# xiyichen/smplify-x-partial

Measured on AMD Instinct MI355X. Metric: fitted frames/sec, higher is better.
Workload: dtype f32; 1 GPU; configs[1]: 256 synthetic frames/GPU, body-only K=25, camera + 5-stage L-BFGS (fit_smplx_smplifyx.yaml, use_vposer=False); frames_per_gpu=256, lbs_mode=dense, gemm_columns_per_gpu=256, parallelism=frames sharded, dp1, closure_evals_per_frame_max=4429, non_finite=0

## Files before the change

smplify-x-partial_amd/csrc/closure_body.h:

```cpp
#pragma once
#include "closure_math.h"
#include "closure_lds.h"
#pragma clang fp contract(on)

#define MARK(i) do { if (D.dbg && blockIdx.x == 0 && threadIdx.x == 0 && D.dbg[62] <= D.dbg[61]) { D.dbg[i] = clock64(); \
        if ((i) == 0) D.dbg[17] = wall_clock64(); if ((i) == 16) D.dbg[18] = wall_clock64(); } } while (0)

#define FOR_CT(w, N) _Pragma("unroll") for (int w##_i = 0; w##_i < ((N) + CT - 1) / CT; ++w##_i)             \
                         if (const int w = t + w##_i * CT; w < (N))

struct NoUpstream {};
struct ExtUpstream {
    const float* djoints;
    int has_dverts;
    float* gc;
};

template <class LDS, class SW, class EXT = NoUpstream>
__device__ __forceinline__ void closure_body(LDS& S, const DevModel& M, const BatchDev& D,
                                             const VarList* __restrict__ vls, const SW* __restrict__ sws,
                                             const ClosureArgs& args, const int b, typename LDS::real_t* gflat,
                                             typename LDS::real_t* fout, const EXT& ext = EXT{}) {
    using Real = typename LDS::real_t;
    constexpr bool F64 = std::is_same<Real, double>::value;
    constexpr bool kExt = !std::is_same<EXT, NoUpstream>::value;
    static_assert(!kExt || !F64, "the external-upstream sweep is fp32");
    constexpr int CT = LDS::kThreads;
    const int t = threadIdx.x;
    const int lane = t & 63, wv = t >> 6;
    const ParLayout& L = D.L;
    const BatchCfgDev& C = D.cfg;

    const bool self_uvp = !F64 && args.use_dense_verts == 2 && M.n_uniq > 0 && M.n_uniq <= LDS::kMaxItems;
    const int stage = __builtin_amdgcn_readfirstlane((args.stage_override != -2) ? args.stage_override : D.stage[b]);
    if constexpr (!kExt) { if (stage >= C.n_stages && !args.forward_only) return; }
    const bool cam_stage = (stage < 0);
    const SW sw = (kExt || cam_stage || args.forward_only) ? SW{} : sws[stage];

    const int cls = (kExt || cam_stage || args.forward_only) ? 2 : ((sw.face_jw != 0.f) ? 2 : ((sw.hand_jw != 0.f) ? 1 : 0));
    const int KL = __builtin_amdgcn_readfirstlane(cls == 2 ? M.K : C.kl[cls]);
    const int NIL = __builtin_amdgcn_readfirstlane(cls == 2 ? M.n_items : C.nil[cls]);

    MARK(0);
    constexpr bool HAS_VP = !std::is_same<decltype(S.V), EmptyLDS>::value;
    constexpr int RIF = (LDS::kMaxItems <= SFX_SMALL_ITEMS) ? SFX_RIF_SMALL : SFX_RIF_BIG;
    constexpr int FWD_PREFIX = (int)(offsetof(LDS, vp) / sizeof(float));
    static_assert(F64 || (FWD_PREFIX % 4 == 0 && FWD_PREFIX + 96 + 2 * VP_H + 128 + 64 <= SFX_FWD_N), "forward-state blob layout");
    static_assert(offsetof(LDS, Ad) % sizeof(fwd_t) == 0 && offsetof(LDS, cd) % sizeof(fwd_t) == 0, "forward-precision members");
    const bool reuse = !F64 && args.reuse_fwd != 0;
    float* fwd = D.fwd ? D.fwd + (size_t)b * SFX_FWD_N : nullptr;
    const Real* xsrc;
// ... 12 lines not shown
    lds_fill_async<CT>(S.vt, M.item_vt, ns * 3);
    lds_fill_async<CT>(S.wj, M.item_wj, ns * SFX_NW); lds_fill_async<CT>(S.ww, M.item_ww, ns * SFX_NW);
    if (M.n_sj <= LDS::kMaxItems * SFX_NW) {
        lds_fill_async<CT>(S.sjs, M.sj_start, SFX_J + 1);
        lds_fill_async<CT>(S.sji, M.sj_item, M.n_sj); lds_fill_async<CT>(S.sjw, M.sj_w, M.n_sj);
    }
    }
    if (reuse) {
        static_assert(F64 || offsetof(LDS, lut_row) == offsetof(LDS, lh45) + 2 * SFX_NHAND * sizeof(float), "hand poses + LUT row are one run");
        lds_fill_async16<CT>(&S, fwd, FWD_PREFIX / 4);
        const float* ex = fwd + FWD_PREFIX;
        lds_fill_async<CT>(S.lh45, ex, 2 * SFX_NHAND + 1);
        if constexpr (HAS_VP) if (C.use_vposer) {
            const float* vx = ex + 96;
            static_assert(offsetof(VposerLDS, h2) == VP_H * sizeof(float) && offsetof(VposerLDS, o) == 2 * VP_H * sizeof(float), "h1 | h2 | o are one run");
            lds_fill_async16<CT>(S.V.h1, vx, (2 * VP_H + 128) / 4);
            lds_fill_async16<CT>(S.V.body, vx + 2 * VP_H + 128, 64 / 4);
        }
    }
    for (int i = t; i < SFX_KD_PAD; i += CT) { if (!reuse) S.feat[i] = 0.f; S.dfeat[i] = 0.f; }
    for (int i = t; i < SFX_NPAR_MAX; i += CT) S.gc[i] = 0.f;
    for (int i = t; i < 168; i += CT) S.dpose[i] = 0.f;
    if constexpr (!F64) {
        if (self_uvp) self_blend_offsets(M.uniq_dirs, M.n_uniq, D.featR + (size_t)args.self_col * SFX_KD_PAD, S.dvert, wv, CT / 64, lane);
    }
    lds_dma_wait();
    __syncthreads();
    const Real* bodypose = S.x + L.emb;
    if constexpr (HAS_VP) {
        if (C.use_vposer && !reuse) {
            vposer_forward<CT>(S.V, M, S.x + L.emb, S.T);
            if (t < 63) D.bodypose[(size_t)b * 63 + t] = S.V.body[t];
        }
        if (C.use_vposer) bodypose = S.V.body;
    }
  if (!reuse) {

    MARK(1);
    if (t < SFX_POSE) {
        Real v;
        if (t < 3) v = S.x[L.go + t];
        else if (t < 66) v = bodypose[t - 3];
        else if (t < 69) v = S.x[L.jaw + t - 66];
        else if (t < 72) v = S.x[L.leye + t - 69];
        else if (t < 75) v = S.x[L.reye + t - 72];
        else {
            const bool left = t < 120;
// ... 91 lines not shown
            for (int q = 0; q < 5; ++q) {
                const Real* Rk = &S.R[chain[q] * 9];
                float o[9];
                for (int i = 0; i < 3; ++i)
                    for (int j = 0; j < 3; ++j)
                        o[i * 3 + j] = Rk[i * 3] * rel[j] + Rk[i * 3 + 1] * rel[3 + j] + Rk[i * 3 + 2] * rel[6 + j];
                for (int e = 0; e < 9; ++e) rel[e] = o[e];
            }
            const float sy = sqrtf(rel[0] * rel[0] + rel[3] * rel[3]);
            const float ang = atan2f(-rel[6], sy);
            float deg = (-ang) * 180.0f / 3.14159265358979323846f;
            deg = fminf(deg, 39.f);
            const int y = (int)rintf(deg);
            row = (y < -39) ? 78 : ((y < 0) ? (39 - y) : y);
        }
        S.lut_row = row;
    }
    __syncthreads();

  }
    MARK(4);
    if (!F64 && args.export_dense) {
        const int slot = D.slot[b];
        if (t < SFX_KD_PAD / 4) reinterpret_cast<float4*>(D.featR_w + (size_t)slot * SFX_KD_PAD)[t] = reinterpret_cast<const float4*>(S.feat)[t];
        MARK(17);
        for (int i = t; i < SFX_J * 12; i += CT) {
            const int j = i / 12, e = i % 12;
            D.AT_w[((size_t)e * SFX_JPAD + j) * D.Bpad + slot] = S.A[i];
        }
        MARK(18);
        if (args.forward_only == 2) {
            if (fwd) {
                const float* sp = reinterpret_cast<const float*>(&S);
                for (int i = t; i < FWD_PREFIX / 4; i += CT)
                    reinterpret_cast<float4*>(fwd)[i] = reinterpret_cast<const float4*>(sp)[i];
                float* ex = fwd + FWD_PREFIX;
                if (t < SFX_NHAND) { ex[t] = S.lh45[t]; ex[SFX_NHAND + t] = S.rh45[t]; }
                if (t == 64) ex[2 * SFX_NHAND] = __int_as_float(S.lut_row);
                if constexpr (HAS_VP) if (C.use_vposer) {
                    float* vx = ex + 96;
                    for (int i = t; i < VP_H; i += CT) { vx[i] = S.V.h1[i]; vx[VP_H + i] = S.V.h2[i]; }
                    if (t < 128) vx[2 * VP_H + t] = S.V.o[t];
                    if (t < 64) vx[2 * VP_H + 128 + t] = S.V.body[t];
                }
            }
            MARK(19);
            return;
        }
    }

    MARK(5);
// ... 604 lines not shown
```

smplify-x-partial_amd/csrc/fused.hip:

```cpp
#include "closure_body.h"
#include "lbfgs_body.h"

#ifndef SFX_SETS_SMALL8
#define SFX_SETS_SMALL8 3
#endif
#ifndef SFX_TICK_OCC
#define SFX_TICK_OCC 2
#endif

template <class LDS>
__global__ __launch_bounds__(LDS::kThreads, LDS::kBlocksPerCU)
void k_fit_rows(DevModel M, BatchDev D, const VarList* __restrict__ vls, const StageW* __restrict__ sws,
                int first_stage, int last_stage, int max_ticks) {
    __shared__ LDS S;
    __shared__ float gflat[SFX_NVAR_MAX];
    __shared__ float fval;
    __shared__ float s_al[SFX_HIST_MAX + 2 * LB_BS];
    __shared__ OptScal st;
    const int b = blockIdx.x;
    ClosureArgs a{};
    a.stage_override = -2;
    for (int it = 0; it < max_ticks; ++it) {
        if (D.stage[b] > last_stage) break;
        closure_body(S, M, D, vls, sws, a, b, gflat, &fval);
// ... 67 lines not shown
            if (D.pen_want && threadIdx.x == 0) D.pen_want[D.slot[b]] = 0;
            copy_operand_column(D, D.slot[b], CTK);
            return;
        }
    }
    const int stage_now = (PF && has_eval) ? s_stage : D.stage[b];
    if (D.pen_want && threadIdx.x == 0) {
        const int st_ = stage_now;
        D.pen_want[D.slot[b]] = (st_ >= 0 && st_ < D.cfg.n_stages) ? (sws[st_].coll > 0.f ? 1 : 0) : 0;
    }
    ClosureArgs e{};
    e.stage_override = -2; e.export_dense = 1; e.forward_only = 2; e.keep_tables = has_eval;
    if (PF && has_eval) { e.stage_override = stage_now; e.x_lds = s_pf + NVEC * SFX_NVAR_MAX + SFX_NPAR_MAX; }
    closure_body(S, M, D, vls, sws, e, b, nullptr, nullptr);
    if (D.dbg && b == 0 && threadIdx.x == 0 && D.dbg[62] <= D.dbg[61]) D.dbg[26] = clock64();
    if (D.dbg && threadIdx.x == 0) {
        const long long dt = wall_clock64() - wc0;
        atomicMax((unsigned long long*)&D.dbg[58], (unsigned long long)dt);
        atomicAdd((unsigned long long*)&D.dbg[59], (unsigned long long)dt);
        atomicAdd((unsigned long long*)&D.dbg[60], 1ull);
    }
}

__global__ __launch_bounds__(256)
void k_uvp_self(DevModel M, BatchDev D, float* __restrict__ out) {
    const int col = blockIdx.x;
    self_blend_offsets(M.uniq_dirs, M.n_uniq, D.featR + (size_t)col * SFX_KD_PAD, out + (size_t)col * M.n_uniq * 3,
                       threadIdx.x >> 6, 4, threadIdx.x & 63);
}
void launch_uvp_self(const DevModel& M, const BatchDev& D, float* out, hipStream_t s) {
    if (D.cfg.B <= 0 || M.n_uniq <= 0) return;
    hipLaunchKernelGGL(k_uvp_self, dim3(D.cfg.B), dim3(256), 0, s, M, D, out);
}

void launch_fit_rows(const DevModel& M, const BatchDev& D, const VarList* vl_dev, const StageW* sw_dev,
                     int first_stage, int last_stage, int max_ticks, hipStream_t s) {
    if (sfx_small_closure(M, D))
        hipLaunchKernelGGL(k_fit_rows<FrameLDSSmall>, dim3(D.cfg.B), dim3(FrameLDSSmall::kThreads), 0, s, M, D, vl_dev, sw_dev, first_stage, last_stage, max_ticks);
    else
        hipLaunchKernelGGL(k_fit_rows<FrameLDS>, dim3(D.cfg.B), dim3(FrameLDS::kThreads), 0, s, M, D, vl_dev, sw_dev, first_stage, last_stage, max_ticks);
}
void launch_tick_dense(const DevModel& M, const BatchDev& D, const VarList* vl_dev, const StageW* sw_dev,
                       int first_stage, int last_stage, int has_eval, hipStream_t s) {
    const int grid = D.act ? D.nrun : D.cfg.B;
    if (grid <= 0) return;
    static const int n_cu = [] { hipDeviceProp_t p; int dev = 0; (void)hipGetDevice(&dev); return hipGetDeviceProperties(&p, dev) == hipSuccess ? p.multiProcessorCount : 256; }();
    if (sfx_small_closure(M, D)) {
#ifdef SFX_LAB
        static const bool t256 = [] { const char* e = getenv("SFX_TICK_THREADS"); return e && atoi(e) == 256; }();
#else
        constexpr bool t256 = false;
#endif
        if (grid <= n_cu && !t256)
            hipLaunchKernelGGL((k_tick_dense<FrameLDSSmall8, 1>), dim3(grid), dim3(FrameLDSSmall8::kThreads), 0, s, M, D, vl_dev, sw_dev, first_stage, last_stage, has_eval);
        else if (grid <= n_cu)
            hipLaunchKernelGGL((k_tick_dense<FrameLDSSmall, 1>), dim3(grid), dim3(FrameLDSSmall::kThreads), 0, s, M, D, vl_dev, sw_dev, first_stage, last_stage, has_eval);
        else
            hipLaunchKernelGGL((k_tick_dense<FrameLDSSmall, SFX_TICK_OCC>), dim3(grid), dim3(FrameLDSSmall::kThreads), 0, s, M, D, vl_dev, sw_dev, first_stage, last_stage, has_eval);
    } else
        hipLaunchKernelGGL((k_tick_dense<FrameLDS, 1>), dim3(grid), dim3(FrameLDS::kThreads), 0, s, M, D, vl_dev, sw_dev, first_stage, last_stage, has_eval);
}
```

smplify-x-partial_amd/csrc/host/batch.hip:

```cpp
#include "host.h"

#include <cmath>
#include <memory>

static void build_layout(ParLayout& L, int NB, int NE, int NPCA, int use_vposer, int latent) {
    L.NB = NB; L.NE = NE; L.NPCA = NPCA;
    L.cam_t = 0; L.go = 3; L.betas = 6; L.lh = L.betas + NB; L.rh = L.lh + NPCA; L.expr = L.rh + NPCA;
    L.jaw = L.expr + NE; L.leye = L.jaw + 3; L.reye = L.leye + 3; L.bodyp = L.reye + 3;
    L.has_bodyp = use_vposer ? 0 : 1;
    L.emb = L.bodyp + (L.has_bodyp ? 63 : 0);
    L.NEMB = use_vposer ? latent : 63;
    L.npar = L.emb + L.NEMB;
}

static void add_group(VarList& v, int off, int len, int has) {
    const int g = v.ngroups++;
    v.g_off[g] = (short)v.n; v.g_len[g] = (short)len; v.g_has[g] = (short)has;
    for (int i = 0; i < len; ++i, ++v.n) if (v.n < SFX_NVAR_MAX) v.idx[v.n] = (short)(off + i);
}

template <class W, class S>
static std::vector<W> stage_weights(const S* st, int n, bool coll) {
    using T = decltype(W::bpw);
    std::vector<W> out(std::max(1, n));
// ... 78 lines not shown
    D.X = b->mem.zeros<float>((size_t)B * SFX_NPAR_MAX);
    D.Xt = b->mem.zeros<float>((size_t)B * SFX_NPAR_MAX);
    if (b->f64) {
        D.X64 = b->mem.zeros<double>((size_t)B * SFX_NPAR_MAX);
        D.Xt64 = b->mem.zeros<double>((size_t)B * SFX_NPAR_MAX);
        D.f64 = b->mem.zeros<double>(B);
        D.g64 = b->mem.zeros<double>((size_t)B * SFX_NVAR_MAX);
        D.cam64 = b->mem.zeros<double>((size_t)B * 8);
    }
    D.gt = b->mem.zeros<float>((size_t)B * K * 2);
    D.conf = b->mem.zeros<float>((size_t)B * K);
    D.jw = b->mem.zeros<float>((size_t)B * K);
    D.cmask = b->mem.zeros<float>((size_t)B * K);
    D.cam = b->mem.zeros<float>((size_t)B * 8);
    D.camR = b->mem.zeros<float>((size_t)B * 9);
    D.regpose = b->mem.zeros<float>((size_t)B * 63);
    D.fd = b->mem.zeros<float>((size_t)B * FD_N);
    D.f = b->mem.zeros<float>(B);
    D.g = b->mem.zeros<float>((size_t)B * SFX_NVAR_MAX);
    D.bodypose = b->mem.zeros<float>((size_t)B * 63);
    D.featR = b->mem.zeros<float>((size_t)SFX_KD_PAD * D.Bpad);
    D.AT = b->mem.zeros<float>((size_t)12 * SFX_JPAD * D.Bpad);
    D.featR_w = D.featR; D.AT_w = D.AT;
    if (c->lbs_mode == 1 && !D.cfg.pen) {
        for (int i = 0; i < 2; ++i) {
            b->featR_o[i] = b->mem.zeros<float>((size_t)SFX_KD_PAD * D.Bpad);
            b->AT_o[i] = b->mem.zeros<float>((size_t)12 * SFX_JPAD * D.Bpad);
        }
    }
    D.verts = b->mem.zeros<float>((size_t)B * m->M.V * 3);
    D.fwd = b->mem.zeros<float>((size_t)B * SFX_FWD_N);
    D.uvp = b->mem.zeros<float>((size_t)B * std::max(1, m->M.n_uniq) * 3);
    if (D.cfg.pen) {
        const int F = (int)(m->faces_host.size() / 3);
        const bool parts = !m->segm_host.empty();
        const int pen_cols = (c->slots > 0 && c->slots < B && c->lbs_mode == 1) ? std::min(B, ((c->slots + 31) / 32) * 32) : B;
        const int pen_cap = std::max(1, c->max_collisions);
        b->pen = m->pen_idle.take(pen_cols, pen_cap, m->parts_gen, &b->pen_cols);
        if (b->pen) sfx_pen_reuse(b->pen);
        else {
            int rc = sfx_pen_create(m->M.V, F, m->faces_host.data(), parts ? m->segm_host.data() : nullptr,
                                    parts ? m->parents_host.data() : nullptr, m->ign_host.empty() ? nullptr : m->ign_host.data(),
                                    (int)(m->ign_host.size() / 2), pen_cap, pen_cols, &b->pen);
            if (rc) return rc;
            b->pen_cols = pen_cols;
        }
        b->pen_cap = pen_cap; b->pen_gen = m->parts_gen;
        b->pen_sigma = c->df_cone_height; b->pen_outside = c->penalize_outside ? 1 : 0;
        (void)sfx_pen_set_point2plane(b->pen, c->point2plane);
        D.pen_loss = b->mem.zeros<float>(B);
// ... 263 lines not shown
```

smplify-x-partial_amd/csrc/host/fit_loop.hip:

```cpp
#include "host.h"
#include "../column_pool.h"

#include <chrono>
#include <cstdio>
#include <cstdlib>
#include <cstring>

static long sfx_fit_tick_bound(const BatchCfgDev& c, int first_stage, int last_stage) {
    const long per_step = (long)c.max_eval + std::max(25, (int)c.lbfgs_max_iter) + 1;
    return (long)(last_stage - first_stage + 1) * c.maxiters * std::max(80L, per_step + 7) * 2  * 2  + 64;
}

struct DenseSwitches {
    bool dbg_nact = false, dbg_host = false;
    int rpb = 0, ahead = 0;
    bool ov_on = true, self_on = true, self_in_serial = false;
    int ov_serial = SFX_OV_SERIAL, self_serial = SFX_OV_SELF_SERIAL, self_max = SFX_OV_SELF_MAX;
};
static const DenseSwitches& dense_switches() {
#ifdef SFX_LAB
    static const DenseSwitches w = [] {
        const auto num = [](const char* name, int unset) { const char* e = getenv(name); return e && *e ? atoi(e) : unset; };
        DenseSwitches v;
        v.dbg_nact = getenv("SFX_DEBUG_NACT") != nullptr; v.dbg_host = getenv("SFX_DEBUG_HOST") != nullptr;
        v.rpb = num("SFX_POLL_ROUNDS", 0); v.ahead = num("SFX_POLL_AHEAD", 0);
        v.ov_on = num("SFX_DENSE_OVERLAP", 1) != 0; v.self_on = num("SFX_DENSE_SELF", 1) != 0; v.self_in_serial = num("SFX_DENSE_SELF_SERIAL", 0) != 0;
        v.ov_serial = num("SFX_OVERLAP_SERIAL", SFX_OV_SERIAL); v.self_max = num("SFX_DENSE_SELF_MAX", SFX_OV_SELF_MAX);
        v.self_serial = num("SFX_OVERLAP_SERIAL", SFX_OV_SELF_SERIAL);
        return v;
    }();
#else
    static constexpr DenseSwitches w{};
#endif
    return w;
}

namespace {
struct DenseLoop {
    sfx_batch* const b; const hipStream_t s; const int first_stage, last_stage;
    BatchDev& D = b->D; const DevModel& M = b->m->M; const int B = D.cfg.B;
    bool overlap = false, self_form = false;
    hipEvent_t last_G = nullptr, prev_G = nullptr;
    hipEvent_t last_T = nullptr;
    long ov_i = 0, tick = 0;
    ColumnPool pool;
    int upl = 0, rpb = 8;
    double host_enq_s = 0.0, host_wait_s = 0.0; long host_batches = 0;
    static inline long nact_hist[9] = {};
    void tick_kernel(const char* name, const BatchDev& Dx, int has_eval) {
        ProfScope p(name, s, Dx.nrun);
        launch_tick_dense(M, Dx, b->vl_dev, b->sw_dev, first_stage, last_stage, has_eval, s);
    }
    int join_s2() {
        if (last_G) SFX_CHECK(hipStreamWaitEvent(s, last_G, 0));
        last_G = prev_G = nullptr;
        return 0;
    }
    int upload(const std::vector<int>* fresh) {
        const std::vector<int>& run = pool.run;
        int* h = b->map_host + (size_t)upl * 3 * B; upl = (upl + 1) % SFX_POLL_BUFS;
        memcpy(h, pool.col.data(), (size_t)B * sizeof(int));
        memcpy(h + B, run.data(), run.size() * sizeof(int));
        SFX_CHECK(hipMemcpyAsync(D.slot, h, (size_t)B * sizeof(int), hipMemcpyHostToDevice, s));
        if (!run.empty()) SFX_CHECK(hipMemcpyAsync(b->act_dev, h + B, run.size() * sizeof(int), hipMemcpyHostToDevice, s));
        if (fresh && !fresh->empty()) {
            memcpy(h + 2 * B, fresh->data(), fresh->size() * sizeof(int));
            SFX_CHECK(hipMemcpyAsync(b->act_new_dev, h + 2 * B, fresh->size() * sizeof(int), hipMemcpyHostToDevice, s));
        }
        D.act = b->act_dev; D.nrun = (int)run.size();
        return 0;
    }
    int tick_beside(hipEvent_t e_G, int has_eval) {
        if (prev_G) SFX_CHECK(hipStreamWaitEvent(s, prev_G, 0));
        prev_G = last_G; last_G = e_G;
        BatchDev Dt = D; Dt.featR_w = b->featR_o[0]; Dt.AT_w = b->AT_o[0];
        tick_kernel("tick", Dt, has_eval);
        float* const f = D.featR; D.featR = b->featR_o[0]; b->featR_o[0] = b->featR_o[1]; b->featR_o[1] = f;
        float* const a = D.AT; D.AT = b->AT_o[0]; b->AT_o[0] = b->AT_o[1]; b->AT_o[1] = a;
        D.featR_w = D.featR; D.AT_w = D.AT;
        return 0;
    }
    int round_self() {
        const int k = (int)(ov_i++ % SFX_OV_EVENTS);
        if (!last_G || !last_T) { SFX_CHECK(hipEventRecord(b->ov_ev[0][k], s)); last_T = b->ov_ev[0][k]; }
        SFX_CHECK(hipStreamWaitEvent(b->s2, last_T, 0));
        { ProfScope p("lbs_dense", b->s2, D.nact); launch_lbs_dense(M, D, b->s2); }
        SFX_CHECK(hipEventRecord(b->ov_ev[1][k], b->s2));
        if (int rc = tick_beside(b->ov_ev[1][k], 2)) return rc;
        last_T = b->ov_ev[0][(k + 1) % SFX_OV_EVENTS];
        SFX_CHECK(hipEventRecord(last_T, s));
        return 0;
    }
    int round_key_rest() {
        if (last_T) { if (int rc = join_s2()) return rc; last_T = nullptr; }
        const int k = (int)(ov_i++ % SFX_OV_EVENTS);
        if (b->m->n_key) { ProfScope p("lbs_dense_key", s, D.nact); launch_lbs_dense_list(M, D, b->m->tile_key, b->m->n_key, s); }
        SFX_CHECK(hipEventRecord(b->ov_ev[0][k], s));
        SFX_CHECK(hipStreamWaitEvent(b->s2, b->ov_ev[0][k], 0));
        { ProfScope p("lbs_dense", b->s2, D.nact); launch_lbs_dense_list(M, D, b->m->tile_rest, b->m->n_rest, b->s2); }
        SFX_CHECK(hipEventRecord(b->ov_ev[1][k], b->s2));
        return tick_beside(b->ov_ev[1][k], 1);
    }
    int round_serial() {
        if (int rc = join_s2()) return rc;
        last_T = nullptr;
        { ProfScope p("lbs_dense", s, D.nact); launch_lbs_dense(M, D, s); }
        if (int rc = eval_penetration(b, -2, s, true)) return rc;
        tick_kernel("tick", D, (dense_switches().self_in_serial && !b->pen && M.n_uniq <= SFX_OV_SELF_UNIQ) ? 2 : 1);
        return 0;
    }
    int rounds(int buf) {
        const DenseSwitches& sw = dense_switches();
        if (sw.dbg_nact) nact_hist[std::min(8, (D.nact - 1) / 32)] += rpb;
        const auto h0 = std::chrono::steady_clock::now();
        for (int q = 0; q < rpb; ++q, ++tick) {
            const int rc = self_form && D.nact > sw.self_serial && D.nact <= sw.self_max ? round_self()
                         : overlap && D.nact > sw.ov_serial && D.nact <= SFX_OV_MAX      ? round_key_rest() : round_serial();
            if (rc) return rc;
        }
        SFX_CHECK(hipMemcpyAsync(b->stage_host + (size_t)buf * B, D.stage, (size_t)B * sizeof(int), hipMemcpyDeviceToHost, s));
        SFX_CHECK(hipEventRecord(b->poll_ev[buf], s));
        host_enq_s += std::chrono::duration<double>(std::chrono::steady_clock::now() - h0).count(); ++host_batches;
        return 0;
    }
    int poll(int cur, bool& done) {
        const auto w0 = std::chrono::steady_clock::now();
        SFX_CHECK(hipEventSynchronize(b->poll_ev[cur]));
        host_wait_s += std::chrono::duration<double>(std::chrono::steady_clock::now() - w0).count();
        std::vector<int> fresh;
        const bool changed = pool.retire(b->stage_host + (size_t)cur * B, last_stage, fresh);
        done = pool.run.empty();
        if (done || !changed) return 0;
        if (!fresh.empty()) {
            if (int rc = join_s2()) return rc;
            if (int rc = upload(&fresh)) return rc;
            BatchDev Dn = D; Dn.act = b->act_new_dev; Dn.nrun = (int)fresh.size();
            tick_kernel("tick_admit", Dn, 0);
        } else if (ColumnPool::slice_emptied(D.nact, (int)pool.run.size())) {
            D.nact = pool.compact();
            if (int rc = join_s2()) return rc;
            if (int rc = upload(nullptr)) return rc;
            tick_kernel("tick", D, 0);
        } else if (int rc = upload(nullptr)) return rc;
        return 0;
    }
    int run(long max_ticks, bool& done) {
        const DenseSwitches& sw = dense_switches();
        overlap = sw.ov_on && !b->pen && b->featR_o[0] && b->featR_o[1] && b->AT_o[0] && b->AT_o[1];
        if (overlap && !b->s2) {
            int lo = 0, hi = 0;
            SFX_CHECK(hipDeviceGetStreamPriorityRange(&lo, &hi));
            SFX_CHECK(hipStreamCreateWithPriority(&b->s2, hipStreamNonBlocking, lo));
            for (auto& ring : b->ov_ev) for (hipEvent_t& e : ring) SFX_CHECK(hipEventCreateWithFlags(&e, hipEventDisableTiming));
        }
        self_form = overlap && sw.self_on && M.n_uniq <= SFX_OV_SELF_UNIQ;
        {
            struct OvDrain { sfx_batch* b; hipStream_t s;
                             ~OvDrain() { if (b->s2) (void)hipStreamSynchronize(b->s2); (void)hipStreamSynchronize(s); b->D.featR_w = b->D.featR; b->D.AT_w = b->D.AT; } } ov_drain{b, s};
            const int ncol = b->slots > 0 ? std::min(b->slots, B) : B;
            pool.reset(B, ncol);
            D.nact = ncol;
            if (int rc = upload(nullptr)) return rc;
            tick_kernel("tick", D, 0);
            const double wall0 = std::chrono::duration<double>(std::chrono::steady_clock::now().time_since_epoch()).count();
            rpb = std::max(1, std::min(64, sw.rpb > 0 ? sw.rpb : 8));
            const int ahead = std::max(1, std::min(SFX_POLL_BUFS - 1, sw.ahead > 0 ? sw.ahead : (b->pen ? 1 : 3)));
            long q_head = 0, q_next = 0;
            for (; q_next < ahead; ++q_next) if (int rc = rounds((int)(q_next % SFX_POLL_BUFS))) return rc;
            while (!done && tick < max_ticks + (long)rpb * (ahead + 1)) {
                if (int rc = rounds((int)(q_next++ % SFX_POLL_BUFS))) return rc;
                if (int rc = poll((int)(q_head++ % SFX_POLL_BUFS), done)) return rc;
            }
            if (b->s2) SFX_CHECK(hipStreamSynchronize(b->s2));
            SFX_CHECK(hipStreamSynchronize(s));
            D.act = nullptr; D.nrun = 0;
            const double wall = std::chrono::duration<double>(std::chrono::steady_clock::now().time_since_epoch()).count() - wall0;
            loop_host_add(host_enq_s, host_wait_s, wall, (double)host_batches * rpb);
            if (sw.dbg_host)
                fprintf(stderr, "[sfx] host enqueue: %ld batches of rounds, %.1f us of host time per round, %.1f %% of the loop's %.1f ms wall time\n",
                        host_batches, 1e6 * host_enq_s / std::max(1L, host_batches * rpb), 100.0 * host_enq_s / std::max(wall, 1e-9), 1e3 * wall);
            if (sw.dbg_nact) {
                fprintf(stderr, "[sfx] rounds by active columns (<=32, <=64, ..., <=256, more), cumulative:");
                for (int i = 0; i < 9; ++i) fprintf(stderr, " %ld", nact_hist[i]);
                fprintf(stderr, "\n");
            }
        }
        SFX_CHECK(hipGetLastError());
        std::vector<int> id(B);
        for (int i = 0; i < B; ++i) id[i] = i;
// ... 73 lines not shown
```

smplify-x-partial_amd/csrc/host/host.h:

```cpp
#pragma once
#include "../../../include/sfx.h"
#include "../sfx_internal.h"
#include "../collide_host.h"
#include "idle_slot.h"

#include <map>
#include <vector>

struct sfx_model {
    DevModel M{};
    DevAlloc mem;
    std::vector<int> faces_host, segm_host, parents_host, ign_host;
    int NB = 0, NE = 0, NPCA = 0;
    std::vector<int> meta_host;
    const int *tile_key = nullptr, *tile_rest = nullptr;
    int n_key = 0, n_rest = 0;
    sfx_batch* fwd = nullptr;
    int fwd_B = 0;
    IdleSlot<sfx_pen, sfx_pen_destroy> pen_idle;
    int parts_gen = 0;
    ~sfx_model() { sfx_batch_destroy(fwd); pen_idle.drop(); }
};

#define SFX_POLL_BUFS 8
#define SFX_OV_EVENTS 4
#ifndef SFX_OV_MAX
#define SFX_OV_MAX 256
#endif
#ifndef SFX_OV_SERIAL
#define SFX_OV_SERIAL 160
#endif
#ifndef SFX_OV_SELF_SERIAL
#define SFX_OV_SELF_SERIAL 64
#endif
#ifndef SFX_OV_SELF_MAX
#define SFX_OV_SELF_MAX 192
#endif
#define SFX_OV_SELF_UNIQ 16
struct sfx_batch {
    sfx_model* m = nullptr;
    BatchDev D{};
    DevAlloc mem;
    VarList* vl_dev = nullptr;
    StageW* sw_dev = nullptr;
    VarList vl_host[2];
    int* stage_host = nullptr;
    int* map_host = nullptr;
    int* act_dev = nullptr;
    int* act_new_dev = nullptr;
    int slots = 0;
    hipEvent_t poll_ev[SFX_POLL_BUFS] = {};
    float *featR_o[2] = {nullptr, nullptr}, *AT_o[2] = {nullptr, nullptr};
    hipStream_t s2 = nullptr;
    hipEvent_t ov_ev[2][SFX_OV_EVENTS] = {};
    int K = 0;
    sfx_pen* pen = nullptr;
    float pen_sigma = 0.f; int pen_outside = 1;
    int pen_cols = 0, pen_cap = 0, pen_gen = -1;
    std::map<int, hipGraphExec_t> pen_graphs;
    int pen_graph_nodes = 0;
    hipStream_t cap_stream = nullptr;
    int* pen_stats_all = nullptr;
    bool pen_chunked = false;
    bool f64 = false;
    StageW64* sw64_dev = nullptr;
    DevAlloc trace_mem;
    long long* dbg_buf = nullptr;
    float* bwd_gc = nullptr;
    struct { float *vposed, *adj_G, *adj_part, *dfeat, *dA; int* want; } bwd = {};
    ~sfx_batch();
};

int refuse_f64(const sfx_batch* b, const char* fn);
int need_f64(const sfx_batch* b, const char* fn);
bool fp32_exact(const double* v, size_t n);
// ... 16 lines not shown
```

smplify-x-partial_amd/csrc/sfx_internal.h:

```cpp
#pragma once
#include <hip/hip_runtime.h>
#include <stdint.h>
#include <algorithm>
#include <vector>

#define SFX_J 55
#define SFX_POSE (3 * SFX_J)
#define SFX_NHAND 45
#define SFX_MAX_K 144
#define SFX_MAX_ITEMS 240
#define SFX_SMALL_ITEMS 32
#define SFX_MAX_DYN 64
#ifndef SFX_RIF_BIG
#define SFX_RIF_BIG 8
#endif
#ifndef SFX_RIF_SMALL
#define SFX_RIF_SMALL 9
#endif
#ifndef SFX_SMALL_OCC
#define SFX_SMALL_OCC 1
#endif
#define SFX_KD_PAD 512
#define SFX_JPAD 56
#define SFX_DENSE_KC 32
// ... 269 lines not shown
    float*       adj_G;
    int Bpad, Vpad;
};
void launch_pen_adjoint(const DevModel& M, const BatchDev& D, hipStream_t s);
struct LbsGradOut { float *go, *bp, *betas, *expr, *jaw, *leye, *reye, *lh, *rh; };
void launch_adj_prep(const DevModel& M, const BatchDev& D, hipStream_t s);
void launch_closure_ext(const DevModel& M, const BatchDev& D, const VarList* vl_dev, const StageW* sw_dev, const ClosureArgs& a,
                        const float* djoints, int has_dverts, float* gc, hipStream_t s);
void launch_scatter_gc(const BatchDev& D, const float* gc, const LbsGradOut& o, hipStream_t s);
int sfx_adj_slices(const DevModel& M);
void launch_lbs_dense(const DevModel& M, const BatchDev& D, hipStream_t s);
void launch_lbs_dense_list(const DevModel& M, const BatchDev& D, const int* list_dev, int n_list, hipStream_t s);
#ifdef SFX_LAB
extern int g_lbs_dense_form;
#endif
void launch_lbfgs_tick(const DevModel& M, const BatchDev& D, const VarList* vl_dev, int first_stage,
                       int last_stage, int init, int step_mode, hipStream_t s);
size_t sfx_optstate_size();
int debug_two_loop(const float* S, const float* Y, int cnt, int hist_cap, const float* g, float* d_out);
void launch_fit_rows(const DevModel& M, const BatchDev& D, const VarList* vl_dev, const StageW* sw_dev,
                     int first_stage, int last_stage, int max_ticks, hipStream_t s);
void launch_tick_dense(const DevModel& M, const BatchDev& D, const VarList* vl_dev, const StageW* sw_dev,
                       int first_stage, int last_stage, int has_eval, hipStream_t s);
void launch_uvp_self(const DevModel& M, const BatchDev& D, float* out, hipStream_t s);
```

Before: 641.4 frames/s.

## Run several L-BFGS rounds per tick launch with a ring of operand sets

Adds a multi-round tick kernel that runs up to R closure+L-BFGS rounds in one launch when few frames remain active. Each round uses the self-blended vertex offsets and exports its dense operands into its own buffer set. The dense LBS GEMMs for those rounds are then queued on the second stream. A new operand ring with up to 2R+1 buffer sets tracks which GEMM reads which set, replacing the fixed double-buffer swap. The aim is to cut per-round launch and event overhead in the low-occupancy tail. The cost is more device memory, copies to spread the current set when switching modes, and more complex synchronisation.

```diff
diff --git a/smplify-x-partial_amd/csrc/closure_body.h b/smplify-x-partial_amd/csrc/closure_body.h
--- a/smplify-x-partial_amd/csrc/closure_body.h
+++ b/smplify-x-partial_amd/csrc/closure_body.h
@@ -16,17 +16,31 @@
     float* gc;
 };
 
-template <class LDS, class SW, class EXT = NoUpstream>
+struct OwnOperands {
+    __device__ __forceinline__ int tid() const { return threadIdx.x; }
+    __device__ __forceinline__ const float* featR(const BatchDev& D) const { return D.featR; }
+    __device__ __forceinline__ float* featR_w(const BatchDev& D) const { return D.featR_w; }
+    __device__ __forceinline__ float* AT_w(const BatchDev& D) const { return D.AT_w; }
+};
+struct OperandSets {
+    const float* r; float* fw; float* aw; int t;
+    __device__ __forceinline__ int tid() const { return t; }
+    __device__ __forceinline__ const float* featR(const BatchDev&) const { return r; }
+    __device__ __forceinline__ float* featR_w(const BatchDev&) const { return fw; }
+    __device__ __forceinline__ float* AT_w(const BatchDev&) const { return aw; }
+};
+
+template <class LDS, class SW, class EXT = NoUpstream, class OPS = OwnOperands>
 __device__ __forceinline__ void closure_body(LDS& S, const DevModel& M, const BatchDev& D,
                                              const VarList* __restrict__ vls, const SW* __restrict__ sws,
                                              const ClosureArgs& args, const int b, typename LDS::real_t* gflat,
-                                             typename LDS::real_t* fout, const EXT& ext = EXT{}) {
+                                             typename LDS::real_t* fout, const EXT& ext = EXT{}, const OPS ops = OPS{}) {
     using Real = typename LDS::real_t;
     constexpr bool F64 = std::is_same<Real, double>::value;
     constexpr bool kExt = !std::is_same<EXT, NoUpstream>::value;
     static_assert(!kExt || !F64, "the external-upstream sweep is fp32");
     constexpr int CT = LDS::kThreads;
-    const int t = threadIdx.x;
+    const int t = ops.tid();
     const int lane = t & 63, wv = t >> 6;
     const ParLayout& L = D.L;
     const BatchCfgDev& C = D.cfg;
@@ -85,7 +99,7 @@
     for (int i = t; i < SFX_NPAR_MAX; i += CT) S.gc[i] = 0.f;
     for (int i = t; i < 168; i += CT) S.dpose[i] = 0.f;
     if constexpr (!F64) {
-        if (self_uvp) self_blend_offsets(M.uniq_dirs, M.n_uniq, D.featR + (size_t)args.self_col * SFX_KD_PAD, S.dvert, wv, CT / 64, lane);
+        if (self_uvp) self_blend_offsets(M.uniq_dirs, M.n_uniq, ops.featR(D) + (size_t)args.self_col * SFX_KD_PAD, S.dvert, wv, CT / 64, lane);
     }
     lds_dma_wait();
     __syncthreads();
@@ -223,11 +237,11 @@
     MARK(4);
     if (!F64 && args.export_dense) {
         const int slot = D.slot[b];
-        if (t < SFX_KD_PAD / 4) reinterpret_cast<float4*>(D.featR_w + (size_t)slot * SFX_KD_PAD)[t] = reinterpret_cast<const float4*>(S.feat)[t];
+        if (t < SFX_KD_PAD / 4) reinterpret_cast<float4*>(ops.featR_w(D) + (size_t)slot * SFX_KD_PAD)[t] = reinterpret_cast<const float4*>(S.feat)[t];
         MARK(17);
         for (int i = t; i < SFX_J * 12; i += CT) {
             const int j = i / 12, e = i % 12;
-            D.AT_w[((size_t)e * SFX_JPAD + j) * D.Bpad + slot] = S.A[i];
+            ops.AT_w(D)[((size_t)e * SFX_JPAD + j) * D.Bpad + slot] = S.A[i];
         }
         MARK(18);
         if (args.forward_only == 2) {
diff --git a/smplify-x-partial_amd/csrc/fused.hip b/smplify-x-partial_amd/csrc/fused.hip
--- a/smplify-x-partial_amd/csrc/fused.hip
+++ b/smplify-x-partial_amd/csrc/fused.hip
@@ -113,6 +113,68 @@
     }
 }
 
+__global__ __launch_bounds__(FrameLDSSmall8::kThreads, 1)
+void k_tick_dense_multi(DevModel M, BatchDev D, const VarList* __restrict__ vls, const StageW* __restrict__ sws,
+                        int first_stage, int last_stage, TickSets sets, int R) {
+    using LDS = FrameLDSSmall8;
+    constexpr int CTK = LDS::kThreads;
+    __shared__ LDS S;
+    __shared__ float gflat[SFX_NVAR_MAX];
+    __shared__ float fval;
+    __shared__ float s_al[SFX_HIST_MAX + 2 * LB_BS];
+    __shared__ OptScal st;
+    __shared__ __align__(16) float s_pf[2048];
+    __shared__ __align__(16) VarList s_vl[2];
+    __shared__ int s_stage;
+    __shared__ float* s_featR[SFX_TICK_ROUNDS + 1];
+    __shared__ float* s_AT[SFX_TICK_ROUNDS + 1];
+    const int b = D.act ? D.act[blockIdx.x] : blockIdx.x;
+    const int slot = D.slot[b];
+    const int self_col = __builtin_amdgcn_readfirstlane(M.n_uniq > 0 ? slot : 0);
+    const bool stamp = D.dbg && blockIdx.x == 0 && threadIdx.x == 0;
+    if (stamp) { D.dbg[62] += 1; if (D.dbg[62] <= D.dbg[61]) D.dbg[24] = clock64(); }
+    if (threadIdx.x == 0) {
+#pragma unroll
+        for (int q = 0; q <= SFX_TICK_ROUNDS; ++q) { s_featR[q] = sets.featR[q]; s_AT[q] = sets.AT[q]; }
+    }
+    __syncthreads();
+    int r = 0;
+#pragma clang loop unroll(disable)
+    for (bool live = D.stage[b] <= last_stage; live && r < R; ++r) {
+        if (r) __syncthreads();
+        int t = threadIdx.x;
+        asm volatile("" : "+v"(t));
+        const OperandSets ops{s_featR[r], s_featR[r + 1], s_AT[r + 1], t};
+        ClosureArgs a{};
+        a.stage_override = -2; a.use_dense_verts = 2; a.reuse_fwd = 1; a.keep_tables = r > 0; a.self_col = self_col;
+        lds_fill_async16<CTK>(s_pf, D.vec + (size_t)b * NVEC * SFX_NVAR_MAX, NVEC * SFX_NVAR_MAX / 4);
+        lds_fill_async16<CTK>(s_pf + NVEC * SFX_NVAR_MAX, D.X + (size_t)b * SFX_NPAR_MAX, SFX_NPAR_MAX / 4);
+        lds_fill_async16<CTK>(s_pf + NVEC * SFX_NVAR_MAX + SFX_NPAR_MAX, D.Xt + (size_t)b * SFX_NPAR_MAX, SFX_NPAR_MAX / 4);
+        lds_fill_async<CTK>(&st, &(reinterpret_cast<const OptState*>(D.opt) + b)->s, (int)(sizeof(OptScal) / 4));
+        if (r == 0) lds_fill_async<CTK>(s_vl, vls, (int)(2 * sizeof(VarList) / 4));
+        closure_body(S, M, D, vls, sws, a, b, gflat, &fval, NoUpstream{}, ops);
+        __syncthreads();
+        if (t < 64)
+            lbfgs_tick_body<SFX_SETS_SMALL8, true>(M, D, s_vl, first_stage, last_stage, 0, 0, b, t, s_al, st, s_pf, &fval, gflat, &s_stage);
+        __syncthreads();
+        if (stamp && r == 0 && D.dbg[62] <= D.dbg[61]) { D.dbg[25] = clock64(); for (int i = 0; i < 17; ++i) D.dbg[40 + i] = D.dbg[i]; }
+        const int stage_now = s_stage;
+        if (stage_now > last_stage) { live = false; break; }
+        ClosureArgs e{};
+        e.stage_override = stage_now; e.export_dense = 1; e.forward_only = 2; e.keep_tables = 1;
+        e.x_lds = s_pf + NVEC * SFX_NVAR_MAX + SFX_NPAR_MAX;
+        closure_body(S, M, D, vls, sws, e, b, nullptr, nullptr, NoUpstream{}, ops);
+        if (stamp && r == 0 && D.dbg[62] <= D.dbg[61]) D.dbg[26] = clock64();
+    }
+    if (r == R) return;
+    const float4* const f0 = reinterpret_cast<const float4*>(s_featR[r] + (size_t)slot * SFX_KD_PAD);
+    const float* const a0 = s_AT[r];
+    for (int q = r + 1; q <= R; ++q) {
+        if (threadIdx.x < SFX_KD_PAD / 4) reinterpret_cast<float4*>(s_featR[q] + (size_t)slot * SFX_KD_PAD)[threadIdx.x] = f0[threadIdx.x];
+        for (int i = threadIdx.x; i < 12 * SFX_JPAD; i += CTK) s_AT[q][(size_t)i * D.Bpad + slot] = a0[(size_t)i * D.Bpad + slot];
+    }
+}
+
 __global__ __launch_bounds__(256)
 void k_uvp_self(DevModel M, BatchDev D, float* __restrict__ out) {
     const int col = blockIdx.x;
@@ -131,23 +193,38 @@
     else
         hipLaunchKernelGGL(k_fit_rows<FrameLDS>, dim3(D.cfg.B), dim3(FrameLDS::kThreads), 0, s, M, D, vl_dev, sw_dev, first_stage, last_stage, max_ticks);
 }
+enum TickShape { TICK_SMALL8, TICK_SMALL_CU, TICK_SMALL_OCC };
+static TickShape tick_small_shape(int grid) {
+    static const int n_cu = [] { hipDeviceProp_t p; int dev = 0; (void)hipGetDevice(&dev); return hipGetDeviceProperties(&p, dev) == hipSuccess ? p.multiProcessorCount : 256; }();
+#ifdef SFX_LAB
+    static const bool t256 = [] { const char* e = getenv("SFX_TICK_THREADS"); return e && atoi(e) == 256; }();
+#else
+    constexpr bool t256 = false;
+#endif
+    return grid > n_cu ? TICK_SMALL_OCC : t256 ? TICK_SMALL_CU : TICK_SMALL8;
+}
+bool tick_dense_multi_ok(const DevModel& M, const BatchDev& D) {
+    return M.n_uniq > 0 && M.n_uniq <= FrameLDSSmall8::kMaxItems && sfx_small_closure(M, D) && tick_small_shape(D.act ? D.nrun : D.cfg.B) == TICK_SMALL8;
+}
+void launch_tick_dense_multi(const DevModel& M, const BatchDev& D, const VarList* vl_dev, const StageW* sw_dev,
+                             int first_stage, int last_stage, const TickSets& sets, int R, hipStream_t s) {
+    const int grid = D.act ? D.nrun : D.cfg.B;
+    if (grid <= 0 || R <= 0) return;
+    hipLaunchKernelGGL(k_tick_dense_multi, dim3(grid), dim3(FrameLDSSmall8::kThreads), 0, s, M, D, vl_dev, sw_dev, first_stage, last_stage, sets, R);
+}
 void launch_tick_dense(const DevModel& M, const BatchDev& D, const VarList* vl_dev, const StageW* sw_dev,
                        int first_stage, int last_stage, int has_eval, hipStream_t s) {
     const int grid = D.act ? D.nrun : D.cfg.B;
     if (grid <= 0) return;
-    static const int n_cu = [] { hipDeviceProp_t p; int dev = 0; (void)hipGetDevice(&dev); return hipGetDeviceProperties(&p, dev) == hipSuccess ? p.multiProcessorCount : 256; }();
     if (sfx_small_closure(M, D)) {
-#ifdef SFX_LAB
-        static const bool t256 = [] { const char* e = getenv("SFX_TICK_THREADS"); return e && atoi(e) == 256; }();
-#else
-        constexpr bool t256 = false;
-#endif
-        if (grid <= n_cu && !t256)
-            hipLaunchKernelGGL((k_tick_dense<FrameLDSSmall8, 1>), dim3(grid), dim3(FrameLDSSmall8::kThreads), 0, s, M, D, vl_dev, sw_dev, first_stage, last_stage, has_eval);
-        else if (grid <= n_cu)
-            hipLaunchKernelGGL((k_tick_dense<FrameLDSSmall, 1>), dim3(grid), dim3(FrameLDSSmall::kThreads), 0, s, M, D, vl_dev, sw_dev, first_stage, last_stage, has_eval);
-        else
-            hipLaunchKernelGGL((k_tick_dense<FrameLDSSmall, SFX_TICK_OCC>), dim3(grid), dim3(FrameLDSSmall::kThreads), 0, s, M, D, vl_dev, sw_dev, first_stage, last_stage, has_eval);
+        switch (tick_small_shape(grid)) {
+        case TICK_SMALL8:
+            hipLaunchKernelGGL((k_tick_dense<FrameLDSSmall8, 1>), dim3(grid), dim3(FrameLDSSmall8::kThreads), 0, s, M, D, vl_dev, sw_dev, first_stage, last_stage, has_eval); break;
+        case TICK_SMALL_CU:
+            hipLaunchKernelGGL((k_tick_dense<FrameLDSSmall, 1>), dim3(grid), dim3(FrameLDSSmall::kThreads), 0, s, M, D, vl_dev, sw_dev, first_stage, last_stage, has_eval); break;
+        case TICK_SMALL_OCC:
+            hipLaunchKernelGGL((k_tick_dense<FrameLDSSmall, SFX_TICK_OCC>), dim3(grid), dim3(FrameLDSSmall::kThreads), 0, s, M, D, vl_dev, sw_dev, first_stage, last_stage, has_eval); break;
+        }
     } else
         hipLaunchKernelGGL((k_tick_dense<FrameLDS, 1>), dim3(grid), dim3(FrameLDS::kThreads), 0, s, M, D, vl_dev, sw_dev, first_stage, last_stage, has_eval);
 }
diff --git a/smplify-x-partial_amd/csrc/host/batch.hip b/smplify-x-partial_amd/csrc/host/batch.hip
--- a/smplify-x-partial_amd/csrc/host/batch.hip
+++ b/smplify-x-partial_amd/csrc/host/batch.hip
@@ -124,10 +124,12 @@
     D.featR = b->mem.zeros<float>((size_t)SFX_KD_PAD * D.Bpad);
     D.AT = b->mem.zeros<float>((size_t)12 * SFX_JPAD * D.Bpad);
     D.featR_w = D.featR; D.AT_w = D.AT;
+    b->op_f[0] = D.featR; b->op_a[0] = D.AT;
     if (c->lbs_mode == 1 && !D.cfg.pen) {
-        for (int i = 0; i < 2; ++i) {
-            b->featR_o[i] = b->mem.zeros<float>((size_t)SFX_KD_PAD * D.Bpad);
-            b->AT_o[i] = b->mem.zeros<float>((size_t)12 * SFX_JPAD * D.Bpad);
+        b->n_sets = (m->M.n_uniq > 0 && m->M.n_uniq <= SFX_OV_SELF_UNIQ && sfx_small_closure(m->M, D)) ? OperandRing::kMaxSets : 3;
+        for (int i = 1; i < b->n_sets; ++i) {
+            b->op_f[i] = b->mem.zeros<float>((size_t)SFX_KD_PAD * D.Bpad);
+            b->op_a[i] = b->mem.zeros<float>((size_t)12 * SFX_JPAD * D.Bpad);
         }
     }
     D.verts = b->mem.zeros<float>((size_t)B * m->M.V * 3);
diff --git a/smplify-x-partial_amd/csrc/host/fit_loop.hip b/smplify-x-partial_amd/csrc/host/fit_loop.hip
--- a/smplify-x-partial_amd/csrc/host/fit_loop.hip
+++ b/smplify-x-partial_amd/csrc/host/fit_loop.hip
@@ -16,6 +16,7 @@
     int rpb = 0, ahead = 0;
     bool ov_on = true, self_on = true, self_in_serial = false;
     int ov_serial = SFX_OV_SERIAL, self_serial = SFX_OV_SELF_SERIAL, self_max = SFX_OV_SELF_MAX;
+    int multi_max = SFX_OV_MULTI_MAX, multi_R = SFX_OV_MULTI_R;
 };
 static const DenseSwitches& dense_switches() {
 #ifdef SFX_LAB
@@ -27,6 +28,8 @@
         v.ov_on = num("SFX_DENSE_OVERLAP", 1) != 0; v.self_on = num("SFX_DENSE_SELF", 1) != 0; v.self_in_serial = num("SFX_DENSE_SELF_SERIAL", 0) != 0;
         v.ov_serial = num("SFX_OVERLAP_SERIAL", SFX_OV_SERIAL); v.self_max = num("SFX_DENSE_SELF_MAX", SFX_OV_SELF_MAX);
         v.self_serial = num("SFX_OVERLAP_SERIAL", SFX_OV_SELF_SERIAL);
+        v.multi_max = num("SFX_DENSE_MULTI", 1) != 0 ? num("SFX_DENSE_MULTI_MAX", getenv("SFX_OVERLAP_SERIAL") ? v.self_serial : SFX_OV_MULTI_MAX) : 0;
+        v.multi_R = num("SFX_DENSE_MULTI_R", SFX_OV_MULTI_R);
         return v;
     }();
 #else
@@ -40,20 +43,26 @@
     sfx_batch* const b; const hipStream_t s; const int first_stage, last_stage;
     BatchDev& D = b->D; const DevModel& M = b->m->M; const int B = D.cfg.B;
     bool overlap = false, self_form = false;
-    hipEvent_t last_G = nullptr, prev_G = nullptr;
+    OperandRing& ring = b->ring;
+    long g_tok = OperandRing::kFree;
     hipEvent_t last_T = nullptr;
     long ov_i = 0, tick = 0;
     ColumnPool pool;
     int upl = 0, rpb = 8;
+    int rot = 0;
+    int multi_R = 1;
     double host_enq_s = 0.0, host_wait_s = 0.0; long host_batches = 0;
     static inline long nact_hist[9] = {};
     void tick_kernel(const char* name, const BatchDev& Dx, int has_eval) {
         ProfScope p(name, s, Dx.nrun);
         launch_tick_dense(M, Dx, b->vl_dev, b->sw_dev, first_stage, last_stage, has_eval, s);
     }
+    hipEvent_t ev_G(long tok) const { return b->ov_ev[1][tok % SFX_OV_EVENTS]; }
+    int wait_G(long tok) { if (tok != OperandRing::kFree) SFX_CHECK(hipStreamWaitEvent(s, ev_G(tok), 0)); return 0; }
+    void point_at_cur() { D.featR = D.featR_w = b->op_f[ring.cur]; D.AT = D.AT_w = b->op_a[ring.cur]; }
     int join_s2() {
-        if (last_G) SFX_CHECK(hipStreamWaitEvent(s, last_G, 0));
-        last_G = prev_G = nullptr;
+        if (int rc = wait_G(g_tok)) return rc;
+        g_tok = OperandRing::kFree; ring.joined();
         return 0;
     }
     int upload(const std::vector<int>* fresh) {
@@ -70,36 +79,37 @@
         D.act = b->act_dev; D.nrun = (int)run.size();
         return 0;
     }
-    int tick_beside(hipEvent_t e_G, int has_eval) {
-        if (prev_G) SFX_CHECK(hipStreamWaitEvent(s, prev_G, 0));
-        prev_G = last_G; last_G = e_G;
-        BatchDev Dt = D; Dt.featR_w = b->featR_o[0]; Dt.AT_w = b->AT_o[0];
+    int tick_beside(long k, int has_eval) {
+        const OperandRing::Write w = ring.next_single();
+        if (int rc = wait_G(w.wait)) return rc;
+        ring.gemm_reads_cur(k); g_tok = k;
+        BatchDev Dt = D; Dt.featR_w = b->op_f[w.set]; Dt.AT_w = b->op_a[w.set];
         tick_kernel("tick", Dt, has_eval);
-        float* const f = D.featR; D.featR = b->featR_o[0]; b->featR_o[0] = b->featR_o[1]; b->featR_o[1] = f;
-        float* const a = D.AT; D.AT = b->AT_o[0]; b->AT_o[0] = b->AT_o[1]; b->AT_o[1] = a;
-        D.featR_w = D.featR; D.AT_w = D.AT;
+        ring.exported(w.set); point_at_cur();
         return 0;
     }
     int round_self() {
-        const int k = (int)(ov_i++ % SFX_OV_EVENTS);
-        if (!last_G || !last_T) { SFX_CHECK(hipEventRecord(b->ov_ev[0][k], s)); last_T = b->ov_ev[0][k]; }
+        const long i = ov_i++;
+        const int k = (int)(i % SFX_OV_EVENTS);
+        if (g_tok == OperandRing::kFree || !last_T) { SFX_CHECK(hipEventRecord(b->ov_ev[0][k], s)); last_T = b->ov_ev[0][k]; }
         SFX_CHECK(hipStreamWaitEvent(b->s2, last_T, 0));
         { ProfScope p("lbs_dense", b->s2, D.nact); launch_lbs_dense(M, D, b->s2); }
         SFX_CHECK(hipEventRecord(b->ov_ev[1][k], b->s2));
-        if (int rc = tick_beside(b->ov_ev[1][k], 2)) return rc;
+        if (int rc = tick_beside(i, 2)) return rc;
         last_T = b->ov_ev[0][(k + 1) % SFX_OV_EVENTS];
         SFX_CHECK(hipEventRecord(last_T, s));
         return 0;
     }
     int round_key_rest() {
         if (last_T) { if (int rc = join_s2()) return rc; last_T = nullptr; }
-        const int k = (int)(ov_i++ % SFX_OV_EVENTS);
+        const long i = ov_i++;
+        const int k = (int)(i % SFX_OV_EVENTS);
         if (b->m->n_key) { ProfScope p("lbs_dense_key", s, D.nact); launch_lbs_dense_list(M, D, b->m->tile_key, b->m->n_key, s); }
         SFX_CHECK(hipEventRecord(b->ov_ev[0][k], s));
         SFX_CHECK(hipStreamWaitEvent(b->s2, b->ov_ev[0][k], 0));
         { ProfScope p("lbs_dense", b->s2, D.nact); launch_lbs_dense_list(M, D, b->m->tile_rest, b->m->n_rest, b->s2); }
         SFX_CHECK(hipEventRecord(b->ov_ev[1][k], b->s2));
-        return tick_beside(b->ov_ev[1][k], 1);
+        return tick_beside(i, 1);
     }
     int round_serial() {
         if (int rc = join_s2()) return rc;
@@ -109,13 +119,55 @@
         tick_kernel("tick", D, (dense_switches().self_in_serial && !b->pen && M.n_uniq <= SFX_OV_SELF_UNIQ) ? 2 : 1);
         return 0;
     }
+    int launch_multi(int n) {
+        const long i = ov_i++;
+        const int k = (int)(i % SFX_OV_EVENTS);
+        const OperandRing::Launch L = ring.next_multi(n, OperandRing::span(multi_R));
+        if (int rc = wait_G(L.wait)) return rc;
+        TickSets ts{};
+        for (int q = 0; q <= n; ++q) { ts.featR[q] = b->op_f[L.set[q]]; ts.AT[q] = b->op_a[L.set[q]]; }
+        { ProfScope p("tick_multi", s, (double)D.nrun * n); launch_tick_dense_multi(M, D, b->vl_dev, b->sw_dev, first_stage, last_stage, ts, n, s); }
+        hipEvent_t const e_P = b->ov_ev[0][(k + 1) % SFX_OV_EVENTS];
+        SFX_CHECK(hipEventRecord(e_P, s));
+        SFX_CHECK(hipStreamWaitEvent(b->s2, e_P, 0));
+        for (int q = 0; q < n; ++q) {
+            BatchDev Dg = D; Dg.featR = ts.featR[q]; Dg.AT = ts.AT[q];
+            ProfScope p("lbs_dense", b->s2, D.nact); launch_lbs_dense(M, Dg, b->s2);
+        }
+        SFX_CHECK(hipEventRecord(b->ov_ev[1][k], b->s2));
+        g_tok = i;
+        ring.launched_multi(L, i); point_at_cur();
+        return 0;
+    }
+    int spread_cur(int n_rot) {
+        for (int i = 0; i < n_rot; ++i) {
+            if (i == ring.cur) continue;
+            SFX_CHECK(hipMemcpyAsync(b->op_f[i], b->op_f[ring.cur], (size_t)SFX_KD_PAD * D.Bpad * sizeof(float), hipMemcpyDeviceToDevice, s));
+            SFX_CHECK(hipMemcpyAsync(b->op_a[i], b->op_a[ring.cur], (size_t)12 * SFX_JPAD * D.Bpad * sizeof(float), hipMemcpyDeviceToDevice, s));
+        }
+        return 0;
+    }
     int rounds(int buf) {
         const DenseSwitches& sw = dense_switches();
         if (sw.dbg_nact) nact_hist[std::min(8, (D.nact - 1) / 32)] += rpb;
         const auto h0 = std::chrono::steady_clock::now();
-        for (int q = 0; q < rpb; ++q, ++tick) {
-            const int rc = self_form && D.nact > sw.self_serial && D.nact <= sw.self_max ? round_self()
-                         : overlap && D.nact > sw.ov_serial && D.nact <= SFX_OV_MAX      ? round_key_rest() : round_serial();
+        const bool multi = self_form && D.nact > 0 && D.nact <= sw.multi_max && OperandRing::span(multi_R) <= b->n_sets && tick_dense_multi_ok(M, D);
+        const bool self = !multi && self_form && D.nact > sw.self_serial && D.nact <= sw.self_max;
+        const bool key_rest = !multi && !self && overlap && D.nact > sw.ov_serial && D.nact <= SFX_OV_MAX;
+        const int rot_new = multi ? OperandRing::span(multi_R) : (self || key_rest) ? 3 : 0;
+        if (rot_new != rot && rot_new) {
+            if (int rc = join_s2()) return rc;
+            last_T = nullptr;
+            if (tick > 0) if (int rc = spread_cur(rot_new)) return rc;
+        }
+        rot = rot_new;
+        if (multi) for (int q = 0; q < rpb; q += multi_R) {
+            const int n = std::min(multi_R, rpb - q);
+            if (int rc = launch_multi(n)) return rc;
+            tick += n;
+        }
+        else for (int q = 0; q < rpb; ++q, ++tick) {
+            const int rc = self ? round_self() : key_rest ? round_key_rest() : round_serial();
             if (rc) return rc;
         }
         SFX_CHECK(hipMemcpyAsync(b->stage_host + (size_t)buf * B, D.stage, (size_t)B * sizeof(int), hipMemcpyDeviceToHost, s));
@@ -146,7 +198,7 @@
     }
     int run(long max_ticks, bool& done) {
         const DenseSwitches& sw = dense_switches();
-        overlap = sw.ov_on && !b->pen && b->featR_o[0] && b->featR_o[1] && b->AT_o[0] && b->AT_o[1];
+        overlap = sw.ov_on && !b->pen && b->n_sets >= 3;
         if (overlap && !b->s2) {
             int lo = 0, hi = 0;
             SFX_CHECK(hipDeviceGetStreamPriorityRange(&lo, &hi));
@@ -161,10 +213,13 @@
             pool.reset(B, ncol);
             D.nact = ncol;
             if (int rc = upload(nullptr)) return rc;
+            ring.joined(); point_at_cur();
+            rot = 0;
             tick_kernel("tick", D, 0);
             const double wall0 = std::chrono::duration<double>(std::chrono::steady_clock::now().time_since_epoch()).count();
             rpb = std::max(1, std::min(64, sw.rpb > 0 ? sw.rpb : 8));
             const int ahead = std::max(1, std::min(SFX_POLL_BUFS - 1, sw.ahead > 0 ? sw.ahead : (b->pen ? 1 : 3)));
+            multi_R = OperandRing::rounds_per_launch(sw.multi_R, (long)ahead * rpb);
             long q_head = 0, q_next = 0;
             for (; q_next < ahead; ++q_next) if (int rc = rounds((int)(q_next % SFX_POLL_BUFS))) return rc;
             while (!done && tick < max_ticks + (long)rpb * (ahead + 1)) {
diff --git a/smplify-x-partial_amd/csrc/host/host.h b/smplify-x-partial_amd/csrc/host/host.h
--- a/smplify-x-partial_amd/csrc/host/host.h
+++ b/smplify-x-partial_amd/csrc/host/host.h
@@ -2,6 +2,7 @@
 #include "../../../include/sfx.h"
 #include "../sfx_internal.h"
 #include "../collide_host.h"
+#include "../operand_ring.h"
 #include "idle_slot.h"
 
 #include <map>
@@ -37,6 +38,12 @@
 #define SFX_OV_SELF_MAX 192
 #endif
 #define SFX_OV_SELF_UNIQ 16
+#ifndef SFX_OV_MULTI_MAX
+#define SFX_OV_MULTI_MAX 96
+#endif
+#ifndef SFX_OV_MULTI_R
+#define SFX_OV_MULTI_R SFX_TICK_ROUNDS
+#endif
 struct sfx_batch {
     sfx_model* m = nullptr;
     BatchDev D{};
@@ -50,7 +57,9 @@
     int* act_new_dev = nullptr;
     int slots = 0;
     hipEvent_t poll_ev[SFX_POLL_BUFS] = {};
-    float *featR_o[2] = {nullptr, nullptr}, *AT_o[2] = {nullptr, nullptr};
+    float *op_f[OperandRing::kMaxSets] = {}, *op_a[OperandRing::kMaxSets] = {};
+    int n_sets = 1;
+    OperandRing ring;
     hipStream_t s2 = nullptr;
     hipEvent_t ov_ev[2][SFX_OV_EVENTS] = {};
     int K = 0;
diff --git a/smplify-x-partial_amd/csrc/operand_ring.h b/smplify-x-partial_amd/csrc/operand_ring.h
--- /dev/null
+++ b/smplify-x-partial_amd/csrc/operand_ring.h
@@ -0,0 +1,36 @@
+#pragma once
+
+struct OperandRing {
+    static constexpr int kMaxRounds = 8, kMaxSets = 2 * kMaxRounds + 1;
+    static constexpr long kFree = -1;
+    int cur = 0;
+    long reader[kMaxSets];
+    OperandRing() { joined(); }
+    void joined() { for (long& r : reader) r = kFree; }
+    void gemm_reads_cur(long e) { reader[cur] = e; }
+
+    struct Write { int set; long wait; };
+    Write next_single() const { const int t = cur < 3 ? (cur + 1) % 3 : 0; return {t, reader[t]}; }
+    void exported(int set) { reader[set] = kFree; cur = set; }
+
+    struct Launch { int n; int set[kMaxRounds + 1]; long wait; };
+    Launch next_multi(int n, int span) const {
+        Launch L{n, {cur}, kFree};
+        const int base = cur < span ? cur : span - 1;
+        for (int q = 1; q <= n; ++q) {
+            L.set[q] = (base + q) % span;
+            if (reader[L.set[q]] > L.wait) L.wait = reader[L.set[q]];
+        }
+        return L;
+    }
+    void launched_multi(const Launch& L, long e) {
+        for (int q = 0; q < L.n; ++q) reader[L.set[q]] = e;
+        cur = L.set[L.n];
+    }
+    static int span(int R) { return 2 * R + 1; }
+    static int rounds_per_launch(int want, long lag_rounds) {
+        long r = want < 1 ? 1 : (want > kMaxRounds ? kMaxRounds : want);
+        if (2 * r > lag_rounds) r = lag_rounds / 2;
+        return r < 1 ? 1 : (int)r;
+    }
+};
diff --git a/smplify-x-partial_amd/csrc/sfx_internal.h b/smplify-x-partial_amd/csrc/sfx_internal.h
--- a/smplify-x-partial_amd/csrc/sfx_internal.h
+++ b/smplify-x-partial_amd/csrc/sfx_internal.h
@@ -315,4 +315,9 @@
                      int first_stage, int last_stage, int max_ticks, hipStream_t s);
 void launch_tick_dense(const DevModel& M, const BatchDev& D, const VarList* vl_dev, const StageW* sw_dev,
                        int first_stage, int last_stage, int has_eval, hipStream_t s);
+#define SFX_TICK_ROUNDS 8
+struct TickSets { float* featR[SFX_TICK_ROUNDS + 1]; float* AT[SFX_TICK_ROUNDS + 1]; };
+bool tick_dense_multi_ok(const DevModel& M, const BatchDev& D);
+void launch_tick_dense_multi(const DevModel& M, const BatchDev& D, const VarList* vl_dev, const StageW* sw_dev,
+                             int first_stage, int last_stage, const TickSets& sets, int R, hipStream_t s);
 void launch_uvp_self(const DevModel& M, const BatchDev& D, float* out, hipStream_t s);
```

After: 677.7 frames/s (median of 6 runs). 5.7% higher.
